# elun15/Graph-Convolutional-Network-for-Multi-Camera-Vehicle-Tracking

Measured on NVIDIA B200. Metric: mpn_inference_directed_edges_per_sec, higher is better.
Workload: dtype f32

## Files before the change

graph-convolutional-network-for-multi-camera-vehicle-tracking_b200/csrc/mpn_forward.cu:

```cuda
#include <mutex>
#include <new>
#include <stdlib.h>
#include <string.h>

#include "common.cuh"
#include "kernels.h"
#include "tcgen05.cuh"

namespace mpn {

enum {
  FC_ENC1_W = 0,
  FC_ENC1_C = 8,
  FC_ENC2_W = 12,
  FC_ENC2_C = 28,
  FC_EDGE_WE = 32,
  FC_BN3_S = 48,
  FC_BN3_T = 52,
  FC_NODE_WE = 64,
  FC_BN4_S = 192,
  FC_BN4_T = 224,
  FC_CLS_W = 256,
  FC_CLS_B = 264,
  FC_EDGE_WE0 = 272,
// ... 745 lines not shown
  const int nwarps = (gridDim.x * SWEEP_THREADS) >> 5;
  const int n_tasks = *g.n_tasks;
  int cur_gid = -1;
  for (int t = gwarp; t < n_tasks; t += nwarps) {
    const TaskRange tr = task_range(g, t);
    if (BATCHED) {
      const int gid = g.node_gid[tr.row];
      if (gid != cur_gid) {
        warp_load_consts(sc, consts + (size_t)gid * FC_TOTAL, lane);
#pragma unroll
        for (int i = lane; i < 64; i += 32) {
          const int p = i >> 2, k = i & 3;
          w2s[p][k] = pack2(sc.v[FC_NODE_WE + 4 * (2 * p) + k], sc.v[FC_NODE_WE + 4 * (2 * p + 1) + k]);
        }
        __syncwarp();
        cur_gid = gid;
      }
    }
    const float4 ps = (YSRC == 0) ? Ps[tr.row] : make_float4(0.f, 0.f, 0.f, 0.f);
    const float a_mine = fmaf(sc.v[FC_BN4_S + lane], A[(size_t)tr.row * MPN_DH + lane], sc.v[FC_BN4_T + lane]);
    f32x2 ap[16], acc[16];
#pragma unroll
    for (int p = 0; p < 16; ++p) {
      ap[p] = pack2(__shfl_sync(0xffffffffu, a_mine, 2 * p), __shfl_sync(0xffffffffu, a_mine, 2 * p + 1));
      acc[p] = 0ull;
    }
    EdgeLoad<U> cur, nxt;
    load_edges<U, YSRC == 0, YSRC == 0, YSRC == 1>(cur, g, tr.beg, tr.end, lane, edge_attr, Pd, ybuf);
    for (int base = tr.beg; base < tr.end; base += 32 * U) {
      const int nbase = base + 32 * U;
      if (nbase < tr.end) load_edges<U, YSRC == 0, YSRC == 0, YSRC == 1>(nxt, g, nbase, tr.end, lane, edge_attr, Pd, ybuf);
      float ep[U][4];
      f32x2 ed[U][4];
#pragma unroll
      for (int j = 0; j < U; ++j) {
        eprime_of<YSRC>(sc, ps, cur.ea[j], cur.pd[j], cur.y[j], ep[j]);
#pragma unroll
        for (int k = 0; k < 4; ++k) ed[j][k] = pack2(ep[j][k], ep[j][k]);
      }
#pragma unroll
      for (int p = 0; p < 16; ++p) {
        ulonglong2 wa, wb;
        asm volatile("ld.shared.v2.b64 {%0, %1}, [%2];" : "=l"(wa.x), "=l"(wa.y) : "r"(w2_addr + p * 32));
        asm volatile("ld.shared.v2.b64 {%0, %1}, [%2];" : "=l"(wb.x), "=l"(wb.y) : "r"(w2_addr + p * 32 + 16));
#pragma unroll
        for (int j = 0; j < U; ++j) {
          f32x2 z = fma2(wa.x, ed[j][0], ap[p]);
          z = fma2(wa.y, ed[j][1], z);
          z = fma2(wb.x, ed[j][2], z);
          z = fma2(wb.y, ed[j][3], z);
          z = relu2(z);
          if (cur.ok[j]) {
            if (AGGMAX) {
              float zl, zh, al, ah;
              unpack2(z, zl, zh);
              unpack2(acc[p], al, ah);
              acc[p] = pack2(fmaxf(al, zl), fmaxf(ah, zh));
            } else {
              acc[p] = add2(acc[p], z);
            }
          }
        }
      }
#pragma unroll
      for (int j = 0; j < U; ++j)
        if (cur.ok[j]) classify_store<CLASSIFY>(sc, ep[j], cur.e[j], logits, pred, prob1);
#pragma unroll
      for (int j = 0; j < U; ++j) {
        cur.e[j] = nxt.e[j];
        cur.ok[j] = nxt.ok[j];
        if (YSRC == 0) { cur.ea[j] = nxt.ea[j]; cur.pd[j] = nxt.pd[j]; }
        else cur.y[j] = nxt.y[j];
      }
    }
    float accf[32];
#pragma unroll
    for (int p = 0; p < 16; ++p) unpack2(acc[p], accf[2 * p], accf[2 * p + 1]);
    const float total = transpose_reduce32<AGGMAX>(accf, lane);
    msg_task[(size_t)t * MPN_DH + lane] = total;
  }
}

constexpr int ATC_THREADS = 128;
constexpr int ATC_CTAS_PER_SM = 5;
constexpr int ATC_SEG = 128;
constexpr int ATC_BATCHES = 512;
constexpr int ATC_NB = 2;
constexpr int ATC_D = 4;
constexpr int ATC_RL = ATC_D + 1;
constexpr int ATC_SLOT_BYTES = 128 * 16;
__device__ __forceinline__ int tile_off(int row, int kcore) { return (row >> 3) * 64 + kcore * 32 + (row & 7) * 4; }
constexpr int ATC_GROUP_BYTES = 3 * 128;
constexpr int ATC_TILE_BYTES = 16 * ATC_GROUP_BYTES;
__device__ __forceinline__ void split_tf32(float v, float& hi, float& lo) {
  hi = __uint_as_float((__float_as_uint(v) + 0x1000u) & 0xffffe000u);
  lo = v - hi;
}
template <int BYTES>
__device__ __forceinline__ void cp_async(void* smem_dst, const void* gsrc) {
  asm volatile("cp.async.ca.shared.global [%0], [%1], %2;" ::"r"(smem_u32(smem_dst)), "l"(gsrc), "n"(BYTES) : "memory");
}
__device__ __forceinline__ void cp_async_commit() { asm volatile("cp.async.commit_group;" ::: "memory"); }
template <int N>
__device__ __forceinline__ void cp_async_wait() { asm volatile("cp.async.wait_group %0;" ::"n"(N) : "memory"); }
__device__ __forceinline__ uint32_t opaque_u32(uint32_t v) {
  asm volatile("" : "+r"(v));
  return v;
}
__device__ __forceinline__ void sts128(uint32_t addr, float a, float b, float c, float d) {
  asm volatile("st.shared.v4.f32 [%0], {%1, %2, %3, %4};" ::"r"(addr), "f"(a), "f"(b), "f"(c), "f"(d) : "memory");
}
__device__ __forceinline__ float4 lds128(uint32_t addr) {
  float4 v;
  asm volatile("ld.shared.v4.f32 {%0, %1, %2, %3}, [%4];" : "=f"(v.x), "=f"(v.y), "=f"(v.z), "=f"(v.w) : "r"(addr) : "memory");
  return v;
}

template <bool CLASSIFY, bool DECIDE, bool AGGMAX, int CTAS>
__global__ void __launch_bounds__(ATC_THREADS, CTAS) apply_tc_kernel(
    const mpn_graph g, const float4* __restrict__ ybuf, const float* __restrict__ A, const float* __restrict__ consts,
    float* __restrict__ msg_task, float2* __restrict__ logits, uint8_t* __restrict__ pred, float* __restrict__ prob1) {
  pdl_wait();
  __shared__ EdgeConsts sc;
  __shared__ __align__(128) float et[2 * ATC_NB][ATC_TILE_BYTES / 4];
  __shared__ __align__(128) float w1[32 * 8];
  __shared__ __align__(128) float w2[32 * 8];
  __shared__ __align__(16) float4 ring[ATC_RL][ATC_THREADS];
  __shared__ int s_row[ATC_SEG], s_beg[ATC_SEG], s_end[ATC_SEG];
  __shared__ int s_bstart[ATC_BATCHES], s_nbatch;
  __shared__ float red[2][ATC_THREADS / 32][32];
  __shared__ __align__(8) uint64_t bar;
  __shared__ uint32_t tmem_slot;
  load_consts(sc, consts);
  const int tid = threadIdx.x, lane = tid & 31, warp = tid >> 5;
  if (warp == 0) tmem_alloc(&tmem_slot, 32 * ATC_NB);
  if (tid == 0) {
    mbar_init(&bar, 1);
    asm volatile("fence.mbarrier_init.release.cluster;" ::: "memory");
  }
  if (tid < 32) {
    float wh[4], wl[4];
#pragma unroll
    for (int k = 0; k < 4; ++k) {
      split_tf32(sc.v[FC_NODE_WE + 4 * tid + k], wh[k], wl[k]);
      uint32_t lb;
      asm("cvt.rna.tf32.f32 %0, %1;" : "=r"(lb) : "f"(wl[k]));
      wl[k] = __uint_as_float(lb);
    }
    *reinterpret_cast<float4*>(&w1[tile_off(tid, 0)]) = make_float4(wh[0], wh[1], wh[2], wh[3]);
    *reinterpret_cast<float4*>(&w1[tile_off(tid, 1)]) = make_float4(wh[0], wh[1], wh[2], wh[3]);
    *reinterpret_cast<float4*>(&w2[tile_off(tid, 0)]) = make_float4(wl[0], wl[1], wl[2], wl[3]);
    *reinterpret_cast<float4*>(&w2[tile_off(tid, 1)]) = make_float4(0.f, 0.f, 0.f, 0.f);
  }
  tc_fence_before();
  __syncthreads();
  tc_fence_after();
  const uint32_t tmem = tmem_slot;
  constexpr uint32_t IDESC = make_idesc_tf32(128, 32);
  const uint64_t d_w1 = make_smem_desc_noswizzle(smem_u32(w1), 128, 256), d_w2 = make_smem_desc_noswizzle(smem_u32(w2), 128, 256);
  const uint64_t d_e1 = make_smem_desc_noswizzle(smem_u32(et[0]), 128, ATC_GROUP_BYTES);
  const uint64_t d_e2 = make_smem_desc_noswizzle(smem_u32(et[0]) + 128, 128, ATC_GROUP_BYTES);
  constexpr uint64_t BUF_STEP = ATC_TILE_BYTES >> 4;
  const uint32_t my_tmem = opaque_u32(tmem + ((uint32_t)(warp * 32) << 16));
  const uint32_t et_addr = opaque_u32(smem_u32(et[0]) + (uint32_t)((tid >> 3) * ATC_GROUP_BYTES + (tid & 7) * 16));
  const uint32_t ring_addr = opaque_u32(smem_u32(&ring[0][tid]));
  constexpr uint32_t TILE_BYTES = ATC_TILE_BYTES;
#pragma unroll
  for (int i = 0; i < 2 * ATC_NB; ++i)
    sts128(et_addr + (uint32_t)i * TILE_BYTES + 256, 1.f, 1.f, 0.f, 0.f);
  uint32_t phase = 0;
  const int n_tasks = *g.n_tasks;
  const int per = (n_tasks + (int)gridDim.x - 1) / (int)gridDim.x;
  const int t_first = blockIdx.x * per, t_last = min(n_tasks, t_first + per);
  const float bn_s = sc.v[FC_BN4_S + lane], bn_t = sc.v[FC_BN4_T + lane];
  const float s3[4] = {sc.v[FC_BN3_S], sc.v[FC_BN3_S + 1], sc.v[FC_BN3_S + 2], sc.v[FC_BN3_S + 3]};
  const float t3[4] = {sc.v[FC_BN3_T], sc.v[FC_BN3_T + 1], sc.v[FC_BN3_T + 2], sc.v[FC_BN3_T + 3]};
  int flushes = 0;

  const int seg_tasks = min(ATC_SEG, ATC_BATCHES / max(1, g.chunk / ATC_THREADS));
  for (int s0 = t_first; s0 < t_last; s0 += seg_tasks) {
    const int ns = min(seg_tasks, t_last - s0);
    __syncthreads();
    for (int i = tid; i < ns; i += ATC_THREADS) {
      const TaskRange tr = task_range(g, s0 + i);
      s_row[i] = tr.row; s_beg[i] = tr.beg; s_end[i] = tr.end;
    }
    __syncthreads();
    for (int i = tid; i < ns; i += ATC_THREADS) {
      int first = 0;
      for (int k = 0; k < i; ++k) first += (s_end[k] - s_beg[k] + ATC_THREADS - 1) / ATC_THREADS;
      const int nb_i = (s_end[i] - s_beg[i] + ATC_THREADS - 1) / ATC_THREADS;
      for (int k = 0; k < nb_i; ++k) s_bstart[first + k] = s_beg[i] + k * ATC_THREADS;
      if (i == ns - 1) s_nbatch = first + nb_i;
    }
    __syncthreads();
    const int n_batch = s_nbatch, seg_last = s_end[ns - 1] - 1;
    int st_j = 0, st_off = 0;
    auto issue_stream = [&]() {
      if (st_j < n_batch) {
        asm volatile("cp.async.ca.shared.global [%0], [%1], 16;" ::"r"(ring_addr + (uint32_t)st_off), "l"(ybuf + min(s_bstart[st_j] + tid, seg_last)) : "memory");
        ++st_j;
        st_off = (st_off == (ATC_RL - 1) * ATC_SLOT_BYTES) ? 0 : st_off + ATC_SLOT_BYTES;
      }
      cp_async_commit();
    };
#pragma unroll
    for (int j = 0; j < ATC_D; ++j) issue_stream();
    float acc[32];
#pragma unroll
    for (int c = 0; c < 32; ++c) acc[c] = 0.f;
    int pending = 0;
    int run_first = 0;
    int c_off = 0, buf = 0, issuer = 0;
    bool ok_prev[ATC_NB];
#pragma unroll
    for (int h = 0; h < ATC_NB; ++h) ok_prev[h] = false;
    float a_next = __ldg(A + (size_t)s_row[0] * MPN_DH + lane);
    auto drain = [&]() {
      mbar_wait(&bar, phase);
      phase ^= 1;
      tc_fence_after();
#pragma unroll
      for (int h = 0; h < ATC_NB; ++h) {
        if (h < pending) {
          float v[32];
          tmem_ld32(my_tmem + 32 * h, v);
          if (ok_prev[h]) {
#pragma unroll
            for (int c = 0; c < 32; ++c) acc[c] = AGGMAX ? fmaxf(acc[c], v[c]) : acc[c] + fabsf(v[c]);
          }
        }
      }
      tc_fence_before();
    };
    auto flush_to_red = [&]() {
      const float total = transpose_reduce32<AGGMAX>(acc, lane);
      red[flushes & 1][warp][lane] = total;
#pragma unroll
      for (int c = 0; c < 32; ++c) acc[c] = 0.f;
    };
    auto store_run = [&](int first, int last_t) {
      const float (*r)[32] = red[flushes & 1];
      msg_task[(size_t)(s0 + last_t) * MPN_DH + lane] = AGGMAX ? fmaxf(fmaxf(r[0][lane], r[1][lane]), fmaxf(r[2][lane], r[3][lane]))
                                                               : (r[0][lane] + r[1][lane]) + (r[2][lane] + r[3][lane]);
      for (int t = first; t < last_t; ++t) msg_task[(size_t)(s0 + t) * MPN_DH + lane] = 0.f;
    };
    for (int ti = 0; ti < ns; ++ti) {
      const int row = s_row[ti], t_beg = s_beg[ti], t_end = s_end[ti];
      const bool new_run = ti == 0 || row != s_row[ti - 1];
      const float a_cur = a_next;
      if (ti + 1 < ns) a_next = __ldg(A + (size_t)s_row[ti + 1] * MPN_DH + lane);
      for (int pos = t_beg; pos < t_end; pos += ATC_NB * ATC_THREADS) {
        const int nb = (pos + ATC_THREADS < t_end) ? ATC_NB : 1;
        bool ok[ATC_NB];
        float ep[ATC_NB][4];
#pragma unroll
        for (int h = 0; h < ATC_NB; ++h) {
          ok[h] = false;
          if (h < nb) {
            cp_async_wait<ATC_D - 1>();
            const float4 yv = lds128(ring_addr + (uint32_t)c_off);
            c_off = (c_off == (ATC_RL - 1) * ATC_SLOT_BYTES) ? 0 : c_off + ATC_SLOT_BYTES;
            issue_stream();
            const int e = pos + h * ATC_THREADS + tid;
            ok[h] = e < t_end;
            ep[h][0] = fmaxf(fmaf(s3[0], yv.x, t3[0]), 0.f);
            ep[h][1] = fmaxf(fmaf(s3[1], yv.y, t3[1]), 0.f);
            ep[h][2] = fmaxf(fmaf(s3[2], yv.z, t3[2]), 0.f);
            ep[h][3] = fmaxf(fmaf(s3[3], yv.w, t3[3]), 0.f);
            if (CLASSIFY && ok[h]) {
              float l0 = sc.v[FC_CLS_B + 0], l1 = sc.v[FC_CLS_B + 1];
#pragma unroll
              for (int k = 0; k < 4; ++k) {
                l0 = fmaf(sc.v[FC_CLS_W + k], ep[h][k], l0);
                l1 = fmaf(sc.v[FC_CLS_W + 4 + k], ep[h][k], l1);
              }
              logits[e] = make_float2(l0, l1);
              if (DECIDE) {
                pred[e] = (l1 > l0) ? 1 : 0;
                prob1[e] = softmax1(l0, l1);
              }
            }
            float eh[4], el[4];
#pragma unroll
            for (int k = 0; k < 4; ++k) split_tf32(ep[h][k], eh[k], el[k]);
            const uint32_t boff = (uint32_t)(buf * ATC_NB + h) * TILE_BYTES;
            sts128(et_addr + boff, el[0], el[1], el[2], el[3]);
            sts128(et_addr + boff + 128, eh[0], eh[1], eh[2], eh[3]);
          }
        }
        if (pending) drain();
#pragma unroll
        for (int h = 0; h < ATC_NB; ++h) ok_prev[h] = ok[h];
        const bool first_batch = pos == t_beg;
        const bool flushed = first_batch && new_run && ti > 0;
        if (first_batch && new_run) {
          if (ti > 0) flush_to_red();
          if (tid < 32) {
            float ah, al, al_hi, al_lo;
            split_tf32(fmaf(bn_s, a_cur, bn_t), ah, al);
            split_tf32(al, al_hi, al_lo);
            *reinterpret_cast<float4*>(&w2[tile_off(tid, 1)]) = make_float4(ah, al_hi, 0.f, 0.f);
          }
        }
        fence_proxy_async_smem();
        tc_fence_before();
        __syncthreads();
        if (tid == issuer) {
          tc_fence_after();
#pragma unroll
          for (int h = 0; h < ATC_NB; ++h) {
            if (h < nb) {
              umma_tf32(tmem + 32 * h, d_e1 + (uint64_t)(buf * ATC_NB + h) * BUF_STEP, d_w1, IDESC, 0);
              umma_tf32(tmem + 32 * h, d_e2 + (uint64_t)(buf * ATC_NB + h) * BUF_STEP, d_w2, IDESC, 1);
            }
          }
          umma_commit(&bar);
        }
        issuer = (issuer + 32) & (ATC_THREADS - 1);
        pending = nb;
        buf ^= 1;
        if (flushed) {
          if (warp == 0) store_run(run_first, ti - 1);
          ++flushes;
          run_first = ti;
        }
      }
    }
    if (pending) drain();
    flush_to_red();
    __syncthreads();
    if (warp == 0) store_run(run_first, ns - 1);
    ++flushes;
    cp_async_wait<0>();
  }
  tc_fence_before();
  __syncthreads();
  if (warp == 0) {
    tc_fence_after();
    tmem_dealloc(tmem, 32 * ATC_NB);
  }
}

template <int STAGE>
__global__ void __launch_bounds__(SWEEP_THREADS) enc_moments_task_kernel(const mpn_graph g, const float2* __restrict__ edge_attr,
                                                                         const float* __restrict__ consts, const float* __restrict__ small,
                                                                         double* __restrict__ task_part) {
  pdl_wait();
  __shared__ EdgeConsts scs[SWEEP_THREADS / 32];
  __shared__ float w2raw[20];
  if (threadIdx.x < 16) w2raw[threadIdx.x] = small[MPN_W_ENC2_W + threadIdx.x];
  else if (threadIdx.x < 20) w2raw[threadIdx.x] = small[MPN_W_ENC2_B + threadIdx.x - 16];
  __syncthreads();
  const int lane = threadIdx.x & 31;
  EdgeConsts& sc = scs[threadIdx.x >> 5];
  const int gwarp = (blockIdx.x * SWEEP_THREADS + threadIdx.x) >> 5;
  const int nwarps = (gridDim.x * SWEEP_THREADS) >> 5;
  const int n_tasks = *g.n_tasks;
  int cur_gid = -1;
  for (int t = gwarp; t < n_tasks; t += nwarps) {
    const TaskRange tr = task_range(g, t);
    if (STAGE == 1) {
      const int gid = g.node_gid[tr.row];
      if (gid != cur_gid) { warp_load_consts(sc, consts + (size_t)gid * FC_TOTAL, lane); cur_gid = gid; }
    }
    double acc[8] = {0, 0, 0, 0, 0, 0, 0, 0};
    for (int e = tr.beg + lane; e < tr.end; e += 32) {
      const float2 ea = ldg_stream2(edge_attr + e);
      if (STAGE == 0) {
        const double a = ea.x, b = ea.y;
        acc[0] += a; acc[1] += b; acc[2] += a * a; acc[3] += a * b; acc[4] += b * b;
      } else {
        float a1[4], u[4];
        enc_layer1(sc, ea, a1);
        enc_layer2_pre(w2raw, w2raw + 16, a1, u);
#pragma unroll
        for (int k = 0; k < 4; ++k) { const double d = u[k]; acc[k] += d; acc[4 + k] += d * d; }
      }
    }
#pragma unroll
    for (int k = 0; k < 8; ++k) {
      const double v = warp_sum(acc[k]);
      if (lane == 0) task_part[(size_t)t * TASK_PART + k] = v;
    }
  }
}

__global__ void __launch_bounds__(128) graph_finalize_kernel(int stage, const mpn_graph g, const double* __restrict__ task_part,
                                                             const float* __restrict__ A, const float4* __restrict__ s1_task,
                                                             const float* __restrict__ small, double* __restrict__ sums_all,
                                                             float* __restrict__ consts_all, int re_e) {
  pdl_wait();
  __shared__ double red[4][64];
  const int gi = blockIdx.x;
  const int n0 = g.graph_nptr[gi], n1 = g.graph_nptr[gi + 1];
  const int t0 = g.taskptr[n0], t1 = g.taskptr[n1];
  const int lane = threadIdx.x & 31, warp = threadIdx.x >> 5;
  double* sums = sums_all + (size_t)gi * SUMS;
  const int ncols = (stage == MPN_STAGE_NODE) ? 10 : 8;
  const int cbase = (stage == MPN_STAGE_NODE) ? 64 : 0;
  for (int col = warp; col < ncols; col += 4) {
    double v = 0.0;
    for (int t = t0 + lane; t < t1; t += 32) v += task_part[(size_t)t * TASK_PART + col];
    v = warp_sum(v);
    if (lane == 0) sums[cbase + col] = v;
  }
  if (stage == MPN_STAGE_NODE) {
    float w[4];
#pragma unroll
    for (int k = 0; k < 4; ++k) w[k] = small[MPN_W_NODE_W + lane * 36 + 32 + k];
    double m1 = 0.0, m2 = 0.0;
    for (int n = n0 + warp; n < n1; n += 4) {
      const int deg = g.rowptr[n + 1] - g.rowptr[n];
      if (deg == 0) continue;
      double sv[4] = {0, 0, 0, 0};
      for (int t = g.taskptr[n]; t < g.taskptr[n + 1]; ++t) {
        const float4 v = s1_task[t];
        sv[0] += v.x; sv[1] += v.y; sv[2] += v.z; sv[3] += v.w;
      }
      const double a = A[(size_t)n * MPN_DH + lane];
      const double qd = w[0] * sv[0] + w[1] * sv[1] + w[2] * sv[2] + w[3] * sv[3];
      m1 += deg * a + qd;
      m2 += deg * a * a + 2.0 * a * qd;
// ... 631 lines not shown
          if (stored) mpn::launch(edge_moments_kernel<0, true, true>, SWEEP_GRID, SWEEP_THREADS, 0, st, g, ea, Ps4, Pd4, yb, p->consts, tp, make_fin(p, stage, false));
          else mpn::launch(edge_moments_kernel<0, false, true>, SWEEP_GRID, SWEEP_THREADS, 0, st, g, ea, Ps4, Pd4, nullptr, p->consts, tp, make_fin(p, stage, false));
        } else {
          if (p->w.reattach_edges) mpn::launch(edge_moments_kernel<1, true, true, true>, SWEEP_GRID, SWEEP_THREADS, 0, st, g, ea, Ps4, Pd4, yb, p->consts, tp, make_fin(p, stage, false));
          else mpn::launch(edge_moments_kernel<1, true, true>, SWEEP_GRID, SWEEP_THREADS, 0, st, g, ea, Ps4, Pd4, yb, p->consts, tp, make_fin(p, stage, false));
        }
        break;
      case MPN_STAGE_NODE:
        if (stored) mpn::launch(node_moments_sweep_kernel<1, true>, SWEEP_RESIDENT_GRID, SWEEP_THREADS, 0, st, g, ea, Ps4, Pd4, yb, p->consts, (float4*)p->s1_task, tp, p->A, p->w.small, make_fin(p, stage, false));
        else mpn::launch(node_moments_sweep_kernel<0, true>, SWEEP_GRID, SWEEP_THREADS, 0, st, g, ea, Ps4, Pd4, nullptr, p->consts, (float4*)p->s1_task, tp, p->A, p->w.small, make_fin(p, stage, false));
        break;
      case MPN_STAGE_APPLY: {
        const bool classify = logits_out != nullptr;
        float2* lg = (float2*)logits_out;
        MPN_REQUIRE(p->L > 0, "batched graphs need num_enc_steps >= 1");
#define MPN_APPLY_B2(YS, CL, MX) mpn::launch(apply_kernel<YS, CL, true, MX>, SWEEP_GRID, SWEEP_THREADS, 0, st, g, ea, Ps4, Pd4, yb, p->A, p->consts, p->msg_task, lg, pred_out, prob1_out)
#define MPN_APPLY_B(YS, CL) do { if (p->w.node_agg == MPN_AGG_MAX) MPN_APPLY_B2(YS, CL, true); else MPN_APPLY_B2(YS, CL, false); } while (0)
        if (stored) { if (classify) MPN_APPLY_B(1, true); else MPN_APPLY_B(1, false); }
        else        { if (classify) MPN_APPLY_B(0, true); else MPN_APPLY_B(0, false); }
#undef MPN_APPLY_B
#undef MPN_APPLY_B2
        break;
      }
      default:
        MPN_REQUIRE(false, "unknown stage %d", stage);
    }
    MPN_LAUNCH_OK();
    if (stage != MPN_STAGE_APPLY) {
      mpn::launch(graph_finalize_kernel, p->n_graphs, 128, 0, st, stage, g, tp, p->A, (const float4*)p->s1_task, p->w.small, p->sums, p->consts,
                                                         p->w.reattach_edges ? (stored ? 2 : 1) : 0);
      MPN_LAUNCH_OK();
    }
    return MPN_OK;
  }
  switch (stage) {
    case MPN_STAGE_ENC0:
      MPN_CUDA_OK(clear_moment_state(p, st));
      mpn::launch(enc_moments_kernel<0>, flat_grid, SWEEP_THREADS, 0, st, ea, g.n_edges, p->consts, p->w.small, p->partials, make_fin(p, stage, fused),
                  (const int*)nullptr);
      break;
    case MPN_STAGE_ENC1:
      if ((((uintptr_t)ea) & 15) == 0 && g.n_edges >= 2) {
        const long long n_pairs = g.n_edges >> 1;
        const int pgrid = (int)min((long long)kNumSMs * 2, (long long)div_up(n_pairs, SWEEP_THREADS));
        FinArgs pf;
        MPN_TRY(sweep_fin(p, stage, fused, pgrid, st, pf));
        mpn::launch(enc_moments1_packed_kernel, pgrid, SWEEP_THREADS, 0, st, (const float4*)ea, n_pairs, ea, g.n_edges, p->consts, p->w.small,
                    p->partials, pf);
      } else {
        mpn::launch(enc_moments_kernel<1>, flat_grid, SWEEP_THREADS, 0, st, ea, g.n_edges, p->consts, p->w.small, p->partials, make_fin(p, stage, fused),
                    (const int*)nullptr);
      }
      break;
    case MPN_STAGE_EDGE:
      if (step == 1) {
        if (stored) mpn::launch(edge_moments_kernel<0, true, false>, SWEEP_GRID, SWEEP_THREADS, 0, st, g, ea, Ps4, Pd4, yb, p->consts, p->partials, make_fin(p, stage, fused));
        else mpn::launch(edge_moments_kernel<0, false, false>, SWEEP_GRID, SWEEP_THREADS, 0, st, g, ea, Ps4, Pd4, nullptr, p->consts, p->partials, make_fin(p, stage, fused));
      } else {
        if (p->w.reattach_edges) mpn::launch(edge_moments_kernel<1, true, false, true>, SWEEP_GRID, SWEEP_THREADS, 0, st, g, ea, Ps4, Pd4, yb, p->consts, p->partials, make_fin(p, stage, fused));
        else mpn::launch(edge_moments_kernel<1, true, false>, SWEEP_GRID, SWEEP_THREADS, 0, st, g, ea, Ps4, Pd4, yb, p->consts, p->partials, make_fin(p, stage, fused));
      }
      break;
    case MPN_STAGE_NODE: {
      FinArgs nf;
      MPN_TRY(sweep_fin(p, stage, fused, stored ? SWEEP_RESIDENT_GRID : SWEEP_GRID, st, nf));
      if (stored) mpn::launch(node_moments_sweep_kernel<1, false>, SWEEP_RESIDENT_GRID, SWEEP_THREADS, 0, st, g, ea, Ps4, Pd4, yb, p->consts, (float4*)p->s1_task, p->partials, p->A, p->w.small, nf);
      else mpn::launch(node_moments_sweep_kernel<0, false>, SWEEP_GRID, SWEEP_THREADS, 0, st, g, ea, Ps4, Pd4, nullptr, p->consts, (float4*)p->s1_task, p->partials, p->A, p->w.small, nf);
      break;
    }
    case MPN_STAGE_APPLY: {
      const bool classify = logits_out != nullptr;
      float2* lg = (float2*)logits_out;
      if (p->L == 0) {
        MPN_REQUIRE(classify, "L == 0 needs a logits buffer");
        mpn::launch(classify_encoded_kernel, flat_grid, SWEEP_THREADS, 0, st, ea, g.n_edges, p->consts, lg, pred_out, prob1_out);
        break;
      }
      static int apply_tc = -1;
      if (apply_tc < 0) { const char* e = getenv("MPN_APPLY_TC"); apply_tc = e ? atoi(e) : 1; }
      p->msg_abs = 0;
      if (p->use_tc && apply_tc && stored && g.chunk >= ATC_THREADS && (!classify || (pred_out != nullptr) == (prob1_out != nullptr))) {
        const bool agg_max = p->w.node_agg == MPN_AGG_MAX;
        p->msg_abs = agg_max ? 0 : 1;
#define MPN_ATC3(CL, DE, MX, NC) mpn::launch(apply_tc_kernel<CL, DE, MX, NC>, kNumSMs * NC, ATC_THREADS, 0, st, g, yb, p->A, p->consts, p->msg_task, lg, pred_out, prob1_out)
#define MPN_ATC2(CL, DE, MX) MPN_ATC3(CL, DE, MX, ATC_CTAS_PER_SM)
#define MPN_ATC(CL, DE) do { if (agg_max) MPN_ATC2(CL, DE, true); else MPN_ATC2(CL, DE, false); } while (0)
        if (!classify) MPN_ATC(false, false);
        else if (pred_out && prob1_out) MPN_ATC(true, true);
        else MPN_ATC(true, false);
#undef MPN_ATC
#undef MPN_ATC2
#undef MPN_ATC3
        break;
      }
#define MPN_APPLY2(YS, CL, MX) mpn::launch(apply_kernel<YS, CL, false, MX>, SWEEP_GRID, SWEEP_THREADS, 0, st, g, ea, Ps4, Pd4, yb, p->A, p->consts, p->msg_task, lg, pred_out, prob1_out)
#define MPN_APPLY(YS, CL) do { if (p->w.node_agg == MPN_AGG_MAX) MPN_APPLY2(YS, CL, true); else MPN_APPLY2(YS, CL, false); } while (0)
      if (stored) { if (classify) MPN_APPLY(1, true); else MPN_APPLY(1, false); }
      else        { if (classify) MPN_APPLY(0, true); else MPN_APPLY(0, false); }
#undef MPN_APPLY
#undef MPN_APPLY2
      break;
    }
    default:
      MPN_REQUIRE(false, "unknown stage %d", stage);
  }
  MPN_LAUNCH_OK();
  return MPN_OK;
}

int mpn_plan_finalize(mpn_fwd_plan* p, int32_t step, int32_t stage, void* stream) {
  MPN_REQUIRE(p, "finalize: NULL plan");
  (void)step;
  if (p->n_graphs > 1) return MPN_OK;
  mpn::launch(finalize_kernel, 1, FIN_THREADS, 0, (cudaStream_t)stream, make_fin(p, stage, false), 0, 1);
  MPN_LAUNCH_OK();
  return MPN_OK;
}

int mpn_plan_reduce(mpn_fwd_plan* p, int32_t stage, int with_consts, void* stream) {
  MPN_REQUIRE(p, "reduce: NULL plan");
  if (p->n_graphs > 1) return MPN_OK;
  mpn::launch(finalize_kernel, 1, FIN_THREADS, 0, (cudaStream_t)stream, make_fin(p, stage, false), 1, with_consts);
  MPN_LAUNCH_OK();
  return MPN_OK;
}

int mpn_plan_node_finalize(mpn_fwd_plan* p, int32_t step, void* stream) {
  MPN_REQUIRE(p, "node_finalize: NULL plan");
  (void)step;
  mpn::launch(node_finalize_kernel<false>, min(kNumSMs * 8, div_up((long long)p->g.n_nodes * 32, 256)), 256, 0, (cudaStream_t)stream, p->g, p->msg_task, p->h_full, PeerArgs(), abs_fix(p));
  MPN_LAUNCH_OK();
  return MPN_OK;
}

struct SideStream {
  cudaStream_t stream;
  cudaEvent_t fork, join;
};
static SideStream* side_stream() {
  static SideStream table[64];
  static int state[64];
  static std::mutex init_lock;
  int dev = 0;
  if (cudaGetDevice(&dev) != cudaSuccess || dev < 0 || dev >= 64) return nullptr;
  std::lock_guard<std::mutex> hold(init_lock);
  if (state[dev] == 0) {
    SideStream& s = table[dev];
    const bool ok = cudaStreamCreateWithFlags(&s.stream, cudaStreamNonBlocking) == cudaSuccess &&
                    cudaEventCreateWithFlags(&s.fork, cudaEventDisableTiming) == cudaSuccess &&
                    cudaEventCreateWithFlags(&s.join, cudaEventDisableTiming) == cudaSuccess;
    state[dev] = ok ? 1 : -1;
  }
  return state[dev] == 1 ? &table[dev] : nullptr;
}

constexpr int TL_MAX = 24;
static bool g_tl_on = false;
static cudaEvent_t g_tl_ev[TL_MAX];
static const char* g_tl_name[TL_MAX];
static int g_tl_n = 0;
static void tl_mark(const char* name, cudaStream_t st, bool first = false) {
  if (!g_tl_on) return;
  if (first) g_tl_n = 0;
  if (g_tl_n >= TL_MAX) return;
  if (!g_tl_ev[g_tl_n] && cudaEventCreate(&g_tl_ev[g_tl_n]) != cudaSuccess) return;
  if (cudaEventRecord(g_tl_ev[g_tl_n], st) != cudaSuccess) return;
  g_tl_name[g_tl_n++] = name;
}

static int forward_impl(const mpn_graph* g, const mpn_weights* w, const float* x, float* edge_attr_rw, int32_t L, int32_t n_cls,
                        float* logits_out, float* h_out, uint8_t* pred_out, float* prob1_out, int use_tc, void* ws, size_t ws_bytes,
                        void* ef_ws, size_t ef_ws_bytes, void* stream) {
  const float* edge_attr = edge_attr_rw;
  MPN_REQUIRE(g && x && edge_attr && logits_out, "forward: NULL argument");
  MPN_REQUIRE(g->row_offset == 0 && g->n_cols == g->n_nodes, "mpn_forward runs an unsharded graph; use the plan API for row blocks");
// ... 334 lines not shown
```

graph-convolutional-network-for-multi-camera-vehicle-tracking_b200/csrc/tcgen05.cuh:

```cuda
#pragma once
#include <cuda.h>
#include <stdint.h>

namespace mpn {

__device__ __forceinline__ uint32_t smem_u32(const void* p) { return (uint32_t)__cvta_generic_to_shared(p); }

__device__ __forceinline__ void mbar_init(uint64_t* bar, uint32_t count) {
  asm volatile("mbarrier.init.shared::cta.b64 [%0], %1;" ::"r"(smem_u32(bar)), "r"(count));
}
__device__ __forceinline__ void mbar_expect_tx(uint64_t* bar, uint32_t bytes) {
  asm volatile("mbarrier.arrive.expect_tx.shared::cta.b64 _, [%0], %1;" ::"r"(smem_u32(bar)), "r"(bytes) : "memory");
}
__device__ __forceinline__ void mbar_arrive(uint64_t* bar) {
  asm volatile("mbarrier.arrive.shared::cta.b64 _, [%0];" ::"r"(smem_u32(bar)) : "memory");
}
__device__ __forceinline__ bool mbar_try_wait(uint64_t* bar, uint32_t parity) {
  uint32_t ok;
  asm volatile(
      "{\n\t"
      ".reg .pred p;\n\t"
      "mbarrier.try_wait.parity.shared::cta.b64 p, [%1], %2;\n\t"
      "selp.u32 %0, 1, 0, p;\n\t"
      "}" : "=r"(ok) : "r"(smem_u32(bar)), "r"(parity) : "memory");
  return ok != 0;
}
__device__ __forceinline__ void mbar_wait(uint64_t* bar, uint32_t parity) {
  if (mbar_try_wait(bar, parity)) return;
  unsigned long long t0, t1;
  asm volatile("mov.u64 %0, %%globaltimer;" : "=l"(t0));
  while (!mbar_try_wait(bar, parity)) {
    asm volatile("mov.u64 %0, %%globaltimer;" : "=l"(t1));
    if (t1 - t0 > 4000000000ull) __trap();
  }
}
__device__ __forceinline__ void tma_load_2d(const CUtensorMap* map, uint64_t* bar, void* dst, int c0, int c1) {
  asm volatile(
      "cp.async.bulk.tensor.2d.shared::cluster.global.mbarrier::complete_tx::bytes [%0], [%1, {%3, %4}], [%2];" ::"r"(smem_u32(dst)),
      "l"(map), "r"(smem_u32(bar)), "r"(c0), "r"(c1)
      : "memory");
}
__device__ __forceinline__ void umma_tf32(uint32_t tmem_d, uint64_t desc_a, uint64_t desc_b, uint32_t idesc, uint32_t accumulate) {
  asm volatile(
      "{\n\t"
      ".reg .pred p;\n\t"
      "setp.ne.b32 p, %4, 0;\n\t"
      "tcgen05.mma.cta_group::1.kind::tf32 [%0], %1, %2, %3, p;\n\t"
      "}" ::"r"(tmem_d), "l"(desc_a), "l"(desc_b), "r"(idesc), "r"(accumulate)
      : "memory");
}
__device__ __forceinline__ void umma_f16(uint32_t tmem_d, uint64_t desc_a, uint64_t desc_b, uint32_t idesc, uint32_t accumulate) {
  asm volatile(
      "{\n\t"
      ".reg .pred p;\n\t"
      "setp.ne.b32 p, %4, 0;\n\t"
      "tcgen05.mma.cta_group::1.kind::f16 [%0], %1, %2, %3, p;\n\t"
      "}" ::"r"(tmem_d), "l"(desc_a), "l"(desc_b), "r"(idesc), "r"(accumulate)
      : "memory");
}
__device__ __forceinline__ void umma_commit(uint64_t* bar) {
  asm volatile("tcgen05.commit.cta_group::1.mbarrier::arrive::one.shared::cluster.b64 [%0];" ::"r"(smem_u32(bar)) : "memory");
}
__device__ __forceinline__ void tmem_ld32(uint32_t taddr, float (&v)[32]) {
  uint32_t r[32];
  asm volatile(
      "tcgen05.ld.sync.aligned.32x32b.x32.b32 "
      "{%0, %1, %2, %3, %4, %5, %6, %7, %8, %9, %10, %11, %12, %13, %14, %15, "
      "%16, %17, %18, %19, %20, %21, %22, %23, %24, %25, %26, %27, %28, %29, %30, %31}, [%32];"
      : "=r"(r[0]), "=r"(r[1]), "=r"(r[2]), "=r"(r[3]), "=r"(r[4]), "=r"(r[5]), "=r"(r[6]), "=r"(r[7]), "=r"(r[8]), "=r"(r[9]),
        "=r"(r[10]), "=r"(r[11]), "=r"(r[12]), "=r"(r[13]), "=r"(r[14]), "=r"(r[15]), "=r"(r[16]), "=r"(r[17]), "=r"(r[18]),
        "=r"(r[19]), "=r"(r[20]), "=r"(r[21]), "=r"(r[22]), "=r"(r[23]), "=r"(r[24]), "=r"(r[25]), "=r"(r[26]), "=r"(r[27]),
        "=r"(r[28]), "=r"(r[29]), "=r"(r[30]), "=r"(r[31])
      : "r"(taddr));
  asm volatile("tcgen05.wait::ld.sync.aligned;" ::: "memory");
#pragma unroll
  for (int i = 0; i < 32; ++i) v[i] = __uint_as_float(r[i]);
}

__device__ __forceinline__ void tmem_ld32_issue(uint32_t taddr, float (&v)[32]) {
  asm volatile(
      "tcgen05.ld.sync.aligned.32x32b.x32.b32 "
      "{%0, %1, %2, %3, %4, %5, %6, %7, %8, %9, %10, %11, %12, %13, %14, %15, "
      "%16, %17, %18, %19, %20, %21, %22, %23, %24, %25, %26, %27, %28, %29, %30, %31}, [%32];"
      : "=f"(v[0]), "=f"(v[1]), "=f"(v[2]), "=f"(v[3]), "=f"(v[4]), "=f"(v[5]), "=f"(v[6]), "=f"(v[7]), "=f"(v[8]), "=f"(v[9]),
        "=f"(v[10]), "=f"(v[11]), "=f"(v[12]), "=f"(v[13]), "=f"(v[14]), "=f"(v[15]), "=f"(v[16]), "=f"(v[17]), "=f"(v[18]),
        "=f"(v[19]), "=f"(v[20]), "=f"(v[21]), "=f"(v[22]), "=f"(v[23]), "=f"(v[24]), "=f"(v[25]), "=f"(v[26]), "=f"(v[27]),
        "=f"(v[28]), "=f"(v[29]), "=f"(v[30]), "=f"(v[31])
      : "r"(taddr));
}
__device__ __forceinline__ void tmem_ld_wait() { asm volatile("tcgen05.wait::ld.sync.aligned;" ::: "memory"); }

__device__ __forceinline__ void tmem_alloc(uint32_t* slot_smem, uint32_t ncols) {
  asm volatile("tcgen05.alloc.cta_group::1.sync.aligned.shared::cta.b32 [%0], %1;" ::"r"(smem_u32(slot_smem)), "r"(ncols));
  asm volatile("tcgen05.relinquish_alloc_permit.cta_group::1.sync.aligned;");
}
__device__ __forceinline__ void tmem_dealloc(uint32_t taddr, uint32_t ncols) {
  asm volatile("tcgen05.dealloc.cta_group::1.sync.aligned.b32 %0, %1;" ::"r"(taddr), "r"(ncols));
}
__device__ __forceinline__ void tc_fence_before() { asm volatile("tcgen05.fence::before_thread_sync;" ::: "memory"); }
__device__ __forceinline__ void tc_fence_after() { asm volatile("tcgen05.fence::after_thread_sync;" ::: "memory"); }
__device__ __forceinline__ void fence_proxy_async_smem() { asm volatile("fence.proxy.async.shared::cta;" ::: "memory"); }

__device__ __forceinline__ uint64_t make_smem_desc_noswizzle(uint32_t saddr, uint32_t lbo_bytes, uint32_t sbo_bytes) {
  uint64_t d = 0;
  d |= (uint64_t)((saddr & 0x3FFFF) >> 4);
  d |= (uint64_t)(lbo_bytes >> 4) << 16;
  d |= (uint64_t)(sbo_bytes >> 4) << 32;
  d |= (uint64_t)1 << 46;
  return d;
}
__host__ __device__ constexpr uint32_t make_idesc_tf32(int M, int N) {
  return (1u << 4) | (2u << 7) | (2u << 10) | ((uint32_t)(N >> 3) << 17) | ((uint32_t)(M >> 4) << 24);
}

}
```

Baseline: 21.45 billion.

## Warp-specialize tensor-core apply kernel with dedicated MMA issuer and mbarrier pipeline

Adds a fifth warp that only builds the per-task A operand and issues tcgen05 MMAs. The four consumer warps stage edge tiles and drain TMEM accumulators through full/done/empty mbarriers over a 3-deep operand ring and 2 TMEM slots. This replaces the per-batch block-wide __syncthreads and round-robin issuer, aiming to overlap tile production, MMA and TMEM drain. It also caps registers at 80 with 16-column TMEM loads, reads BN3 constants from shared memory, and uses a named barrier for flushes. The cost is more barrier traffic, an extra warp per CTA, and a risk of register spills.

```diff
diff --git a/graph-convolutional-network-for-multi-camera-vehicle-tracking_b200/csrc/mpn_forward.cu b/graph-convolutional-network-for-multi-camera-vehicle-tracking_b200/csrc/mpn_forward.cu
--- a/graph-convolutional-network-for-multi-camera-vehicle-tracking_b200/csrc/mpn_forward.cu
+++ b/graph-convolutional-network-for-multi-camera-vehicle-tracking_b200/csrc/mpn_forward.cu
@@ -851,16 +851,22 @@
 }
 
 constexpr int ATC_THREADS = 128;
+constexpr int ATC_ISSUER = ATC_THREADS / 32;
+constexpr int ATC_BLOCK = ATC_THREADS + 32;
 constexpr int ATC_CTAS_PER_SM = 5;
+constexpr int ATC_S = 2;
+constexpr int ATC_OPS = 3;
+constexpr int ATC_MAX_REGS = 80;
+static_assert(FC_BN3_S % 4 == 0 && FC_BN3_T == FC_BN3_S + 4, "the apply sweep reads [s3 | t3] as two 16-byte shared loads");
 constexpr int ATC_SEG = 128;
 constexpr int ATC_BATCHES = 512;
-constexpr int ATC_NB = 2;
 constexpr int ATC_D = 4;
 constexpr int ATC_RL = ATC_D + 1;
 constexpr int ATC_SLOT_BYTES = 128 * 16;
 __device__ __forceinline__ int tile_off(int row, int kcore) { return (row >> 3) * 64 + kcore * 32 + (row & 7) * 4; }
 constexpr int ATC_GROUP_BYTES = 3 * 128;
 constexpr int ATC_TILE_BYTES = 16 * ATC_GROUP_BYTES;
+constexpr int ATC_W_BYTES = 32 * 8 * 4;
 __device__ __forceinline__ void split_tf32(float v, float& hi, float& lo) {
   hi = __uint_as_float((__float_as_uint(v) + 0x1000u) & 0xffffe000u);
   lo = v - hi;
@@ -884,78 +890,71 @@
   asm volatile("ld.shared.v4.f32 {%0, %1, %2, %3}, [%4];" : "=f"(v.x), "=f"(v.y), "=f"(v.z), "=f"(v.w) : "r"(addr) : "memory");
   return v;
 }
-
-template <bool CLASSIFY, bool DECIDE, bool AGGMAX, int CTAS>
-__global__ void __launch_bounds__(ATC_THREADS, CTAS) apply_tc_kernel(
+__device__ __forceinline__ void atc_consumer_sync() { asm volatile("bar.sync 1, %0;" ::"n"(ATC_THREADS) : "memory"); }
+
+template <bool CLASSIFY, bool DECIDE, bool AGGMAX>
+__global__ void __maxnreg__(ATC_MAX_REGS) apply_tc_kernel(
     const mpn_graph g, const float4* __restrict__ ybuf, const float* __restrict__ A, const float* __restrict__ consts,
     float* __restrict__ msg_task, float2* __restrict__ logits, uint8_t* __restrict__ pred, float* __restrict__ prob1) {
   pdl_wait();
-  __shared__ EdgeConsts sc;
-  __shared__ __align__(128) float et[2 * ATC_NB][ATC_TILE_BYTES / 4];
+  __shared__ __align__(16) EdgeConsts sc;
+  __shared__ __align__(128) float et[ATC_OPS][ATC_TILE_BYTES / 4];
   __shared__ __align__(128) float w1[32 * 8];
-  __shared__ __align__(128) float w2[32 * 8];
+  __shared__ __align__(128) float w2[ATC_OPS][32 * 8];
   __shared__ __align__(16) float4 ring[ATC_RL][ATC_THREADS];
   __shared__ int s_row[ATC_SEG], s_beg[ATC_SEG], s_end[ATC_SEG];
   __shared__ int s_bstart[ATC_BATCHES], s_nbatch;
   __shared__ float red[2][ATC_THREADS / 32][32];
-  __shared__ __align__(8) uint64_t bar;
+  __shared__ __align__(8) uint64_t full[ATC_OPS], done[ATC_S], empty[ATC_S];
   __shared__ uint32_t tmem_slot;
   load_consts(sc, consts);
   const int tid = threadIdx.x, lane = tid & 31, warp = tid >> 5;
-  if (warp == 0) tmem_alloc(&tmem_slot, 32 * ATC_NB);
+  if (warp == 0) tmem_alloc(&tmem_slot, 32 * ATC_S);
   if (tid == 0) {
-    mbar_init(&bar, 1);
+#pragma unroll
+    for (int o = 0; o < ATC_OPS; ++o) mbar_init(&full[o], ATC_THREADS);
+#pragma unroll
+    for (int s = 0; s < ATC_S; ++s) {
+      mbar_init(&done[s], 1);
+      mbar_init(&empty[s], ATC_THREADS);
+    }
     asm volatile("fence.mbarrier_init.release.cluster;" ::: "memory");
   }
-  if (tid < 32) {
+  if (warp == ATC_ISSUER) {
     float wh[4], wl[4];
 #pragma unroll
     for (int k = 0; k < 4; ++k) {
-      split_tf32(sc.v[FC_NODE_WE + 4 * tid + k], wh[k], wl[k]);
+      split_tf32(sc.v[FC_NODE_WE + 4 * lane + k], wh[k], wl[k]);
       uint32_t lb;
       asm("cvt.rna.tf32.f32 %0, %1;" : "=r"(lb) : "f"(wl[k]));
       wl[k] = __uint_as_float(lb);
     }
-    *reinterpret_cast<float4*>(&w1[tile_off(tid, 0)]) = make_float4(wh[0], wh[1], wh[2], wh[3]);
-    *reinterpret_cast<float4*>(&w1[tile_off(tid, 1)]) = make_float4(wh[0], wh[1], wh[2], wh[3]);
-    *reinterpret_cast<float4*>(&w2[tile_off(tid, 0)]) = make_float4(wl[0], wl[1], wl[2], wl[3]);
-    *reinterpret_cast<float4*>(&w2[tile_off(tid, 1)]) = make_float4(0.f, 0.f, 0.f, 0.f);
+    *reinterpret_cast<float4*>(&w1[tile_off(lane, 0)]) = make_float4(wh[0], wh[1], wh[2], wh[3]);
+    *reinterpret_cast<float4*>(&w1[tile_off(lane, 1)]) = make_float4(wh[0], wh[1], wh[2], wh[3]);
+#pragma unroll
+    for (int o = 0; o < ATC_OPS; ++o) *reinterpret_cast<float4*>(&w2[o][tile_off(lane, 0)]) = make_float4(wl[0], wl[1], wl[2], wl[3]);
+    fence_proxy_async_smem();
   }
   tc_fence_before();
   __syncthreads();
   tc_fence_after();
   const uint32_t tmem = tmem_slot;
-  constexpr uint32_t IDESC = make_idesc_tf32(128, 32);
-  const uint64_t d_w1 = make_smem_desc_noswizzle(smem_u32(w1), 128, 256), d_w2 = make_smem_desc_noswizzle(smem_u32(w2), 128, 256);
-  const uint64_t d_e1 = make_smem_desc_noswizzle(smem_u32(et[0]), 128, ATC_GROUP_BYTES);
-  const uint64_t d_e2 = make_smem_desc_noswizzle(smem_u32(et[0]) + 128, 128, ATC_GROUP_BYTES);
-  constexpr uint64_t BUF_STEP = ATC_TILE_BYTES >> 4;
-  const uint32_t my_tmem = opaque_u32(tmem + ((uint32_t)(warp * 32) << 16));
-  const uint32_t et_addr = opaque_u32(smem_u32(et[0]) + (uint32_t)((tid >> 3) * ATC_GROUP_BYTES + (tid & 7) * 16));
-  const uint32_t ring_addr = opaque_u32(smem_u32(&ring[0][tid]));
-  constexpr uint32_t TILE_BYTES = ATC_TILE_BYTES;
-#pragma unroll
-  for (int i = 0; i < 2 * ATC_NB; ++i)
-    sts128(et_addr + (uint32_t)i * TILE_BYTES + 256, 1.f, 1.f, 0.f, 0.f);
-  uint32_t phase = 0;
   const int n_tasks = *g.n_tasks;
   const int per = (n_tasks + (int)gridDim.x - 1) / (int)gridDim.x;
   const int t_first = blockIdx.x * per, t_last = min(n_tasks, t_first + per);
-  const float bn_s = sc.v[FC_BN4_S + lane], bn_t = sc.v[FC_BN4_T + lane];
-  const float s3[4] = {sc.v[FC_BN3_S], sc.v[FC_BN3_S + 1], sc.v[FC_BN3_S + 2], sc.v[FC_BN3_S + 3]};
-  const float t3[4] = {sc.v[FC_BN3_T], sc.v[FC_BN3_T + 1], sc.v[FC_BN3_T + 2], sc.v[FC_BN3_T + 3]};
+  const int seg_tasks = min(ATC_SEG, ATC_BATCHES / max(1, g.chunk / ATC_THREADS));
+  uint32_t it = 0;
   int flushes = 0;
 
-  const int seg_tasks = min(ATC_SEG, ATC_BATCHES / max(1, g.chunk / ATC_THREADS));
   for (int s0 = t_first; s0 < t_last; s0 += seg_tasks) {
     const int ns = min(seg_tasks, t_last - s0);
     __syncthreads();
-    for (int i = tid; i < ns; i += ATC_THREADS) {
+    for (int i = tid; i < ns; i += ATC_BLOCK) {
       const TaskRange tr = task_range(g, s0 + i);
       s_row[i] = tr.row; s_beg[i] = tr.beg; s_end[i] = tr.end;
     }
     __syncthreads();
-    for (int i = tid; i < ns; i += ATC_THREADS) {
+    for (int i = tid; i < ns; i += ATC_BLOCK) {
       int first = 0;
       for (int k = 0; k < i; ++k) first += (s_end[k] - s_beg[k] + ATC_THREADS - 1) / ATC_THREADS;
       const int nb_i = (s_end[i] - s_beg[i] + ATC_THREADS - 1) / ATC_THREADS;
@@ -963,6 +962,49 @@
       if (i == ns - 1) s_nbatch = first + nb_i;
     }
     __syncthreads();
+
+    if (warp == ATC_ISSUER) {
+      constexpr uint32_t IDESC = make_idesc_tf32(128, 32);
+      const uint64_t d_w1 = make_smem_desc_noswizzle(smem_u32(w1), 128, 256), d_w2 = make_smem_desc_noswizzle(smem_u32(w2[0]), 128, 256);
+      const uint64_t d_e1 = make_smem_desc_noswizzle(smem_u32(et[0]), 128, ATC_GROUP_BYTES);
+      const uint64_t d_e2 = make_smem_desc_noswizzle(smem_u32(et[0]) + 128, 128, ATC_GROUP_BYTES);
+      const uint32_t a_addr = smem_u32(&w2[0][tile_off(lane, 1)]);
+      const float bn_s = sc.v[FC_BN4_S + lane], bn_t = sc.v[FC_BN4_T + lane];
+      float a_next = __ldg(A + (size_t)s_row[0] * MPN_DH + lane);
+      for (int ti = 0; ti < ns; ++ti) {
+        const float a_cur = a_next;
+        if (ti + 1 < ns) a_next = __ldg(A + (size_t)s_row[ti + 1] * MPN_DH + lane);
+        float ah, al, al_hi, al_lo;
+        split_tf32(fmaf(bn_s, a_cur, bn_t), ah, al);
+        split_tf32(al, al_hi, al_lo);
+        for (int pos = s_beg[ti]; pos < s_end[ti]; pos += ATC_THREADS, ++it) {
+          const uint32_t s = it % ATC_S, o = it % ATC_OPS;
+          if (it >= ATC_S) mbar_wait(&empty[s], ((it / ATC_S) - 1) & 1);
+          sts128(a_addr + o * ATC_W_BYTES, ah, al_hi, 0.f, 0.f);
+          fence_proxy_async_smem();
+          __syncwarp();
+          if (lane == 0) {
+            mbar_wait(&full[o], (it / ATC_OPS) & 1);
+            tc_fence_after();
+            umma_tf32(tmem + 32 * s, d_e1 + o * (uint64_t)(ATC_TILE_BYTES >> 4), d_w1, IDESC, 0);
+            umma_tf32(tmem + 32 * s, d_e2 + o * (uint64_t)(ATC_TILE_BYTES >> 4), d_w2 + o * (uint64_t)(ATC_W_BYTES >> 4), IDESC, 1);
+            umma_commit(&done[s]);
+          }
+          __syncwarp();
+        }
+      }
+      continue;
+    }
+
+    const uint32_t my_tmem = opaque_u32(tmem + ((uint32_t)(warp * 32) << 16));
+    const uint32_t et_addr = opaque_u32(smem_u32(et[0]) + (uint32_t)((tid >> 3) * ATC_GROUP_BYTES + (tid & 7) * 16));
+    const uint32_t ring_addr = opaque_u32(smem_u32(&ring[0][tid]));
+    if (s0 == t_first) {
+#pragma unroll
+      for (int i = 0; i < ATC_OPS; ++i)
+        sts128(et_addr + (uint32_t)i * ATC_TILE_BYTES + 256, 1.f, 1.f, 0.f, 0.f);
+    }
+    const uint32_t bn3_addr = smem_u32(&sc.v[FC_BN3_S]);
     const int n_batch = s_nbatch, seg_last = s_end[ns - 1] - 1;
     int st_j = 0, st_off = 0;
     auto issue_stream = [&]() {
@@ -978,136 +1020,98 @@
     float acc[32];
 #pragma unroll
     for (int c = 0; c < 32; ++c) acc[c] = 0.f;
-    int pending = 0;
     int run_first = 0;
-    int c_off = 0, buf = 0, issuer = 0;
-    bool ok_prev[ATC_NB];
-#pragma unroll
-    for (int h = 0; h < ATC_NB; ++h) ok_prev[h] = false;
-    float a_next = __ldg(A + (size_t)s_row[0] * MPN_DH + lane);
-    auto drain = [&]() {
-      mbar_wait(&bar, phase);
-      phase ^= 1;
+    int c_off = 0;
+    uint32_t drained = it;
+    uint32_t ok_bits = 0;
+    auto drain_one = [&]() {
+      const uint32_t s = drained % ATC_S;
+      mbar_wait(&done[s], (drained / ATC_S) & 1);
       tc_fence_after();
-#pragma unroll
-      for (int h = 0; h < ATC_NB; ++h) {
-        if (h < pending) {
-          float v[32];
-          tmem_ld32(my_tmem + 32 * h, v);
-          if (ok_prev[h]) {
-#pragma unroll
-            for (int c = 0; c < 32; ++c) acc[c] = AGGMAX ? fmaxf(acc[c], v[c]) : acc[c] + fabsf(v[c]);
+      const bool add = (ok_bits >> (drained % ATC_OPS)) & 1u;
+#pragma unroll
+      for (int h = 0; h < 2; ++h) {
+        float v[16];
+        tmem_ld16(my_tmem + 32 * s + 16 * h, v);
+        if (add) {
+#pragma unroll
+          for (int c = 0; c < 16; ++c)
+            acc[16 * h + c] = AGGMAX ? fmaxf(acc[16 * h + c], v[c]) : acc[16 * h + c] + fabsf(v[c]);
+        }
+      }
+      tc_fence_before();
+      mbar_arrive(&empty[s]);
+      ++drained;
+    };
+    auto flush_run = [&](int first, int last_t) {
+      const float total = transpose_reduce32<AGGMAX>(acc, lane);
+      red[flushes & 1][warp][lane] = total;
+#pragma unroll
+      for (int c = 0; c < 32; ++c) acc[c] = 0.f;
+      atc_consumer_sync();
+      if (warp == 0) {
+        const float (*r)[32] = red[flushes & 1];
+        msg_task[(size_t)(s0 + last_t) * MPN_DH + lane] = AGGMAX ? fmaxf(fmaxf(r[0][lane], r[1][lane]), fmaxf(r[2][lane], r[3][lane]))
+                                                                 : (r[0][lane] + r[1][lane]) + (r[2][lane] + r[3][lane]);
+        for (int t = first; t < last_t; ++t) msg_task[(size_t)(s0 + t) * MPN_DH + lane] = 0.f;
+      }
+      ++flushes;
+    };
+    for (int ti = 0; ti < ns; ++ti) {
+      const int t_beg = s_beg[ti], t_end = s_end[ti];
+      const bool new_run = ti > 0 && s_row[ti] != s_row[ti - 1];
+      for (int pos = t_beg; pos < t_end; pos += ATC_THREADS, ++it) {
+        if (pos == t_beg && new_run) {
+          while (drained != it) drain_one();
+          flush_run(run_first, ti - 1);
+          run_first = ti;
+        }
+        cp_async_wait<ATC_D - 1>();
+        const float4 yv = lds128(ring_addr + (uint32_t)c_off);
+        c_off = (c_off == (ATC_RL - 1) * ATC_SLOT_BYTES) ? 0 : c_off + ATC_SLOT_BYTES;
+        issue_stream();
+        const int e = pos + tid;
+        const bool ok = e < t_end;
+        const float4 s3 = lds128(bn3_addr), t3 = lds128(bn3_addr + 16);
+        float ep[4];
+        ep[0] = fmaxf(fmaf(s3.x, yv.x, t3.x), 0.f);
+        ep[1] = fmaxf(fmaf(s3.y, yv.y, t3.y), 0.f);
+        ep[2] = fmaxf(fmaf(s3.z, yv.z, t3.z), 0.f);
+        ep[3] = fmaxf(fmaf(s3.w, yv.w, t3.w), 0.f);
+        if (CLASSIFY && ok) {
+          float l0 = sc.v[FC_CLS_B + 0], l1 = sc.v[FC_CLS_B + 1];
+#pragma unroll
+          for (int k = 0; k < 4; ++k) {
+            l0 = fmaf(sc.v[FC_CLS_W + k], ep[k], l0);
+            l1 = fmaf(sc.v[FC_CLS_W + 4 + k], ep[k], l1);
+          }
+          logits[e] = make_float2(l0, l1);
+          if (DECIDE) {
+            pred[e] = (l1 > l0) ? 1 : 0;
+            prob1[e] = softmax1(l0, l1);
           }
         }
-      }
-      tc_fence_before();
-    };
-    auto flush_to_red = [&]() {
-      const float total = transpose_reduce32<AGGMAX>(acc, lane);
-      red[flushes & 1][warp][lane] = total;
-#pragma unroll
-      for (int c = 0; c < 32; ++c) acc[c] = 0.f;
-    };
-    auto store_run = [&](int first, int last_t) {
-      const float (*r)[32] = red[flushes & 1];
-      msg_task[(size_t)(s0 + last_t) * MPN_DH + lane] = AGGMAX ? fmaxf(fmaxf(r[0][lane], r[1][lane]), fmaxf(r[2][lane], r[3][lane]))
-                                                               : (r[0][lane] + r[1][lane]) + (r[2][lane] + r[3][lane]);
-      for (int t = first; t < last_t; ++t) msg_task[(size_t)(s0 + t) * MPN_DH + lane] = 0.f;
-    };
-    for (int ti = 0; ti < ns; ++ti) {
-      const int row = s_row[ti], t_beg = s_beg[ti], t_end = s_end[ti];
-      const bool new_run = ti == 0 || row != s_row[ti - 1];
-      const float a_cur = a_next;
-      if (ti + 1 < ns) a_next = __ldg(A + (size_t)s_row[ti + 1] * MPN_DH + lane);
-      for (int pos = t_beg; pos < t_end; pos += ATC_NB * ATC_THREADS) {
-        const int nb = (pos + ATC_THREADS < t_end) ? ATC_NB : 1;
-        bool ok[ATC_NB];
-        float ep[ATC_NB][4];
-#pragma unroll
-        for (int h = 0; h < ATC_NB; ++h) {
-          ok[h] = false;
-          if (h < nb) {
-            cp_async_wait<ATC_D - 1>();
-            const float4 yv = lds128(ring_addr + (uint32_t)c_off);
-            c_off = (c_off == (ATC_RL - 1) * ATC_SLOT_BYTES) ? 0 : c_off + ATC_SLOT_BYTES;
-            issue_stream();
-            const int e = pos + h * ATC_THREADS + tid;
-            ok[h] = e < t_end;
-            ep[h][0] = fmaxf(fmaf(s3[0], yv.x, t3[0]), 0.f);
-            ep[h][1] = fmaxf(fmaf(s3[1], yv.y, t3[1]), 0.f);
-            ep[h][2] = fmaxf(fmaf(s3[2], yv.z, t3[2]), 0.f);
-            ep[h][3] = fmaxf(fmaf(s3[3], yv.w, t3[3]), 0.f);
-            if (CLASSIFY && ok[h]) {
-              float l0 = sc.v[FC_CLS_B + 0], l1 = sc.v[FC_CLS_B + 1];
-#pragma unroll
-              for (int k = 0; k < 4; ++k) {
-                l0 = fmaf(sc.v[FC_CLS_W + k], ep[h][k], l0);
-                l1 = fmaf(sc.v[FC_CLS_W + 4 + k], ep[h][k], l1);
-              }
-              logits[e] = make_float2(l0, l1);
-              if (DECIDE) {
-                pred[e] = (l1 > l0) ? 1 : 0;
-                prob1[e] = softmax1(l0, l1);
-              }
-            }
-            float eh[4], el[4];
-#pragma unroll
-            for (int k = 0; k < 4; ++k) split_tf32(ep[h][k], eh[k], el[k]);
-            const uint32_t boff = (uint32_t)(buf * ATC_NB + h) * TILE_BYTES;
-            sts128(et_addr + boff, el[0], el[1], el[2], el[3]);
-            sts128(et_addr + boff + 128, eh[0], eh[1], eh[2], eh[3]);
-          }
-        }
-        if (pending) drain();
-#pragma unroll
-        for (int h = 0; h < ATC_NB; ++h) ok_prev[h] = ok[h];
-        const bool first_batch = pos == t_beg;
-        const bool flushed = first_batch && new_run && ti > 0;
-        if (first_batch && new_run) {
-          if (ti > 0) flush_to_red();
-          if (tid < 32) {
-            float ah, al, al_hi, al_lo;
-            split_tf32(fmaf(bn_s, a_cur, bn_t), ah, al);
-            split_tf32(al, al_hi, al_lo);
-            *reinterpret_cast<float4*>(&w2[tile_off(tid, 1)]) = make_float4(ah, al_hi, 0.f, 0.f);
-          }
-        }
+        float eh[4], el[4];
+#pragma unroll
+        for (int k = 0; k < 4; ++k) split_tf32(ep[k], eh[k], el[k]);
+        const uint32_t o = it % ATC_OPS;
+        sts128(et_addr + o * ATC_TILE_BYTES, el[0], el[1], el[2], el[3]);
+        sts128(et_addr + o * ATC_TILE_BYTES + 128, eh[0], eh[1], eh[2], eh[3]);
         fence_proxy_async_smem();
-        tc_fence_before();
-        __syncthreads();
-        if (tid == issuer) {
-          tc_fence_after();
-#pragma unroll
-          for (int h = 0; h < ATC_NB; ++h) {
-            if (h < nb) {
-              umma_tf32(tmem + 32 * h, d_e1 + (uint64_t)(buf * ATC_NB + h) * BUF_STEP, d_w1, IDESC, 0);
-              umma_tf32(tmem + 32 * h, d_e2 + (uint64_t)(buf * ATC_NB + h) * BUF_STEP, d_w2, IDESC, 1);
-            }
-          }
-          umma_commit(&bar);
-        }
-        issuer = (issuer + 32) & (ATC_THREADS - 1);
-        pending = nb;
-        buf ^= 1;
-        if (flushed) {
-          if (warp == 0) store_run(run_first, ti - 1);
-          ++flushes;
-          run_first = ti;
-        }
-      }
-    }
-    if (pending) drain();
-    flush_to_red();
-    __syncthreads();
-    if (warp == 0) store_run(run_first, ns - 1);
-    ++flushes;
+        mbar_arrive(&full[o]);
+        ok_bits = (ok_bits & ~(1u << o)) | ((uint32_t)ok << o);
+        if (it + 1 - drained > ATC_S) drain_one();
+      }
+    }
+    while (drained != it) drain_one();
+    flush_run(run_first, ns - 1);
     cp_async_wait<0>();
   }
   tc_fence_before();
   __syncthreads();
   if (warp == 0) {
     tc_fence_after();
-    tmem_dealloc(tmem, 32 * ATC_NB);
+    tmem_dealloc(tmem, 32 * ATC_S);
   }
 }
 
@@ -1905,15 +1909,13 @@
       if (p->use_tc && apply_tc && stored && g.chunk >= ATC_THREADS && (!classify || (pred_out != nullptr) == (prob1_out != nullptr))) {
         const bool agg_max = p->w.node_agg == MPN_AGG_MAX;
         p->msg_abs = agg_max ? 0 : 1;
-#define MPN_ATC3(CL, DE, MX, NC) mpn::launch(apply_tc_kernel<CL, DE, MX, NC>, kNumSMs * NC, ATC_THREADS, 0, st, g, yb, p->A, p->consts, p->msg_task, lg, pred_out, prob1_out)
-#define MPN_ATC2(CL, DE, MX) MPN_ATC3(CL, DE, MX, ATC_CTAS_PER_SM)
+#define MPN_ATC2(CL, DE, MX) mpn::launch(apply_tc_kernel<CL, DE, MX>, kNumSMs * ATC_CTAS_PER_SM, ATC_BLOCK, 0, st, g, yb, p->A, p->consts, p->msg_task, lg, pred_out, prob1_out)
 #define MPN_ATC(CL, DE) do { if (agg_max) MPN_ATC2(CL, DE, true); else MPN_ATC2(CL, DE, false); } while (0)
         if (!classify) MPN_ATC(false, false);
         else if (pred_out && prob1_out) MPN_ATC(true, true);
         else MPN_ATC(true, false);
 #undef MPN_ATC
 #undef MPN_ATC2
-#undef MPN_ATC3
         break;
       }
 #define MPN_APPLY2(YS, CL, MX) mpn::launch(apply_kernel<YS, CL, false, MX>, SWEEP_GRID, SWEEP_THREADS, 0, st, g, ea, Ps4, Pd4, yb, p->A, p->consts, p->msg_task, lg, pred_out, prob1_out)
diff --git a/graph-convolutional-network-for-multi-camera-vehicle-tracking_b200/csrc/tcgen05.cuh b/graph-convolutional-network-for-multi-camera-vehicle-tracking_b200/csrc/tcgen05.cuh
--- a/graph-convolutional-network-for-multi-camera-vehicle-tracking_b200/csrc/tcgen05.cuh
+++ b/graph-convolutional-network-for-multi-camera-vehicle-tracking_b200/csrc/tcgen05.cuh
@@ -77,6 +77,19 @@
   for (int i = 0; i < 32; ++i) v[i] = __uint_as_float(r[i]);
 }
 
+__device__ __forceinline__ void tmem_ld16(uint32_t taddr, float (&v)[16]) {
+  uint32_t r[16];
+  asm volatile(
+      "tcgen05.ld.sync.aligned.32x32b.x16.b32 "
+      "{%0, %1, %2, %3, %4, %5, %6, %7, %8, %9, %10, %11, %12, %13, %14, %15}, [%16];"
+      : "=r"(r[0]), "=r"(r[1]), "=r"(r[2]), "=r"(r[3]), "=r"(r[4]), "=r"(r[5]), "=r"(r[6]), "=r"(r[7]), "=r"(r[8]), "=r"(r[9]),
+        "=r"(r[10]), "=r"(r[11]), "=r"(r[12]), "=r"(r[13]), "=r"(r[14]), "=r"(r[15])
+      : "r"(taddr));
+  asm volatile("tcgen05.wait::ld.sync.aligned;" ::: "memory");
+#pragma unroll
+  for (int i = 0; i < 16; ++i) v[i] = __uint_as_float(r[i]);
+}
+
 __device__ __forceinline__ void tmem_ld32_issue(uint32_t taddr, float (&v)[32]) {
   asm volatile(
       "tcgen05.ld.sync.aligned.32x32b.x32.b32 "
```

New measurement: 19.15 billion, median of 6. -10.7%, worse.
